# CLSFramework/gym-soccer-2d-env

Hardware: AMD Instinct MI355X
Metric: env-steps/sec at 65536 parallel reach_ball envs per MI355X (higher is better)
Workload: dtype f32

## Files before the change

gym-soccer-2d-env_amd/csrc/s2d_device.h:

```cpp
#pragma once
#include <hip/hip_runtime.h>
#include <stdint.h>

#include "../../include/s2d.h"

#define S2D_DEV __device__ __forceinline__

enum { S2D_MODE_DISCRETE = 0, S2D_MODE_CONT1 = 1, S2D_MODE_TURN4 = 2 };

struct S2DHot {
  float inv_half_l, inv_half_w, half_l, half_w;
  float player_decay, ball_decay;
  float player_accel_max2, player_speed_max2, ball_speed_max2, rsum2;
  float stamina_max, stamina_inc_max, extra_stamina, stamina_capacity;
  float recover_init, recover_dec_thr_value, recover_min, recover_dec;
  float effort_init, effort_dec_thr_value, effort_min, effort_dec, effort_inc_thr_value, effort_inc;
  float dash_power_rate, max_dash_power, min_dash_power, max_dash_angle, min_dash_angle;
  float dash_angle_step, inv_dash_angle_step, side_dash_rate, back_dash_rate;
  float min_distance_to_ball, min_dist2_thr, act_scale;
  int max_steps, n_actions, auto_reset;
  uint32_t seed_lo, seed_hi, gid_lo, gid_hi;
  float max_moment, min_moment, inertia_moment, player_rand, ball_rand;
};
struct S2DRare {
  float player_accel_max, player_speed_max, ball_speed_max, rsum, collision_vel_rate;
  float recover_init;
  float ball_position_x, ball_position_y, ball_speed, ball_direction, travel_factor;
  int change_ball_position, change_ball_velocity;
  int tab_len;
  float tab_power;
  int pad[1];
};

S2D_DEV float to_vgpr(float x) {
  float y;
  asm("v_mov_b32 %0, %1" : "=v"(y) : "s"(x));
  return y;
}
S2D_DEV S2DHot hot_in_vgprs(const S2DHot& p) {
  S2DHot v = p;
  v.inv_half_l = to_vgpr(p.inv_half_l); v.inv_half_w = to_vgpr(p.inv_half_w);
  v.half_l = to_vgpr(p.half_l); v.half_w = to_vgpr(p.half_w);
  v.player_decay = to_vgpr(p.player_decay); v.ball_decay = to_vgpr(p.ball_decay);
  v.player_accel_max2 = to_vgpr(p.player_accel_max2); v.player_speed_max2 = to_vgpr(p.player_speed_max2);
  v.ball_speed_max2 = to_vgpr(p.ball_speed_max2); v.rsum2 = to_vgpr(p.rsum2);
  v.stamina_max = to_vgpr(p.stamina_max); v.stamina_inc_max = to_vgpr(p.stamina_inc_max);
  v.extra_stamina = to_vgpr(p.extra_stamina);
  v.recover_dec_thr_value = to_vgpr(p.recover_dec_thr_value); v.recover_min = to_vgpr(p.recover_min);
  v.recover_dec = to_vgpr(p.recover_dec);
  v.effort_init = to_vgpr(p.effort_init); v.effort_dec_thr_value = to_vgpr(p.effort_dec_thr_value);
  v.effort_min = to_vgpr(p.effort_min); v.effort_dec = to_vgpr(p.effort_dec);
  v.effort_inc_thr_value = to_vgpr(p.effort_inc_thr_value); v.effort_inc = to_vgpr(p.effort_inc);
  v.dash_power_rate = to_vgpr(p.dash_power_rate); v.max_dash_power = to_vgpr(p.max_dash_power);
  v.min_dash_power = to_vgpr(p.min_dash_power); v.max_dash_angle = to_vgpr(p.max_dash_angle);
  v.min_dash_angle = to_vgpr(p.min_dash_angle);
  v.inv_dash_angle_step = to_vgpr(p.inv_dash_angle_step);
  v.side_dash_rate = to_vgpr(p.side_dash_rate); v.back_dash_rate = to_vgpr(p.back_dash_rate);
  v.min_distance_to_ball = to_vgpr(p.min_distance_to_ball); v.act_scale = to_vgpr(p.act_scale);
  v.min_dist2_thr = to_vgpr(p.min_dist2_thr);
  return v;
}

enum { S2D_ST_RESET = 0, S2D_ST_POLICY = 1, S2D_ST_SELECT = 2, S2D_ST_NOISE = 3, S2D_ST_NOISE_RESET = 5 };

struct U4 { uint32_t x, y, z, w; };

S2D_DEV U4 philox4x32_10(uint32_t c0, uint32_t c1, uint32_t c2, uint32_t c3, uint32_t k0, uint32_t k1) {
#pragma unroll
  for (int r = 0; r < 10; ++r) {
    uint64_t p0 = (uint64_t)0xD2511F53u * c0;
    uint64_t p1 = (uint64_t)0xCD9E8D57u * c2;
    uint32_t n0 = (uint32_t)(p1 >> 32) ^ c1 ^ k0, n2 = (uint32_t)(p0 >> 32) ^ c3 ^ k1;
    c0 = n0; c1 = (uint32_t)p1; c2 = n2; c3 = (uint32_t)p0;
    k0 += 0x9E3779B9u; k1 += 0xBB67AE85u;
  }
  return U4{c0, c1, c2, c3};
}
S2D_DEV U4 s2d_draw(const S2DHot& p, uint32_t gid_lo, uint32_t gid_hi, uint32_t cycle, uint32_t stream,
                    uint32_t block) {
  return philox4x32_10(gid_lo, gid_hi, cycle, (stream << 16) | block, p.seed_lo, p.seed_hi);
}
S2D_DEV U4 policy_quad(const S2DHot& p, uint32_t gid_lo, uint32_t gid_hi, uint32_t k, uint32_t stream) {
  return s2d_draw(p, gid_lo, gid_hi, k >> 2, stream, 0);
}
S2D_DEV uint32_t quad_word(const U4& q, uint32_t k) {
  uint32_t j = k & 3u;
  uint32_t lo = (j & 1u) ? q.y : q.x, hi = (j & 1u) ? q.w : q.z;
  return (j & 2u) ? hi : lo;
// ... 198 lines not shown
  }
}

S2D_DEV int command_code(float x) {
  int c = S2D_CMD_NONE;
  c = (x >= -1.5f && x <= -0.5f) ? (int)S2D_CMD_FREEZE : c;
  c = (x >= 0.5f && x < 1.5f) ? (int)S2D_CMD_DASH : c;
  c = (x >= 1.5f && x < 2.5f) ? (int)S2D_CMD_TURN : c;
  return c;
}

struct ObsOut { float o[S2D_OBS_DIM]; };

enum { S2D_FLAG_GOAL = 1, S2D_FLAG_OUT = 2, S2D_FLAG_TIMEOUT = 4 };

S2D_DEV int judge(const S2DHot& p, float px, float py, float d2, int step_number, float& dist) {
  dist = sqrt_cr(d2);
  int f = (dist < p.min_distance_to_ball) ? S2D_FLAG_GOAL : 0;
  f |= (fabsf(px) > p.half_l || fabsf(py) > p.half_w) ? S2D_FLAG_OUT : 0;
  f |= (step_number > p.max_steps) ? S2D_FLAG_TIMEOUT : 0;
  return f;
}
S2D_DEV int judge_sq(const S2DHot& p, float px, float py, float d2, int step_number) {
  int f = (d2 < p.min_dist2_thr) ? S2D_FLAG_GOAL : 0;
  f |= (fabsf(px) > p.half_l || fabsf(py) > p.half_w) ? S2D_FLAG_OUT : 0;
  f |= (step_number > p.max_steps) ? S2D_FLAG_TIMEOUT : 0;
  return f;
}
S2D_DEV float observe_player(const S2DHot& p, float px, float py, float body, float bx, float by, float* o) {
  float dx = bx - px, dy = by - py;
  float player_to_ball = atan2_deg(dy, dx);
  float rel = norm_deg(player_to_ball - body);
  o[0] = rel * 0.005555555555555556f;
  o[1] = body * 0.005555555555555556f;
  o[2] = px * p.inv_half_l;
  o[3] = py * p.inv_half_w;
  return rel;
}
S2D_DEV void observe_ball(const S2DHot& p, float bx, float by, float bvx, float bvy, float* o) {
  float ball_speed = hypot2(bvx, bvy);
  float ball_direction = atan2_deg(bvy, bvx);
  o[4] = bx * p.inv_half_l;
  o[5] = by * p.inv_half_w;
  o[6] = ball_speed * 0.3333333333333333f;
  o[7] = ball_direction * 0.002777777777777778f;
  o[8] = bvx * 0.3333333333333333f;
  o[9] = bvy * 0.3333333333333333f;
}
S2D_DEV float observe(const S2DHot& p, float px, float py, float body, float bx, float by, float bvx, float bvy,
                      ObsOut& ob) {
  observe_ball(p, bx, by, bvx, bvy, ob.o);
  return observe_player(p, px, py, body, bx, by, ob.o);
}
S2D_DEV float reward_of(float prev_dist, float prev_angle, float dist, float rel, int flags, int& result) {
  float r = prev_dist - dist;
  r += (fabsf(prev_angle) - fabsf(rel)) * 0.005555555555555556f;
  r = (flags & S2D_FLAG_GOAL) ? r + 10.0f : r;
  r = (flags & S2D_FLAG_OUT) ? r - -10.0f : r;
  r = (flags & S2D_FLAG_TIMEOUT) ? r - 5.0f : r;
  int res = (flags & S2D_FLAG_GOAL) ? S2D_RESULT_GOAL : S2D_RESULT_NONE;
  res = (flags & S2D_FLAG_OUT) ? S2D_RESULT_OUT : res;
  res = (flags & S2D_FLAG_TIMEOUT) ? S2D_RESULT_TIMEOUT : res;
  result = res;
  return r;
}

S2D_DEV void observe_and_check(const S2DHot& p, Env& e, float d2, ObsOut& ob, int& done, float& reward, int& result) {
  float rel = observe(p, e.px, e.py, e.body, e.bx, e.by, e.bvx, e.bvy, ob);
  float dist;
  int flags = judge(p, e.px, e.py, d2, e.step_number, dist);
  reward = reward_of(e.prev_dist, e.prev_angle, dist, rel, flags, result);
  e.prev_dist = dist;
  e.prev_angle = rel;
  done = flags ? 1 : 0;
}

struct CmdPrep { float power, dir, dir_rate; };
S2D_DEV CmdPrep dash_prepare(const S2DHot& p, float power, float dir) {
  power = clampf(power, p.min_dash_power, p.max_dash_power);
  dir = clampf(dir, p.min_dash_angle, p.max_dash_angle);
  float disc = p.dash_angle_step * rintf(dir * p.inv_dash_angle_step);
  dir = (p.dash_angle_step > 0.0f) ? disc : dir;
  float ad = fabsf(dir);
  float r_back = p.back_dash_rate - ((p.back_dash_rate - p.side_dash_rate) * (1.0f - (ad - 90.0f) * 0.011111111111111112f));
  float r_fwd = p.side_dash_rate + ((1.0f - p.side_dash_rate) * (1.0f - ad * 0.011111111111111112f));
  float dir_rate = clampf(ad > 90.0f ? r_back : r_fwd, 0.0f, 1.0f);
  return CmdPrep{power, dir, dir_rate};
}
S2D_DEV void dash_apply(const S2DHot& p, Env& e, const CmdPrep& c, float& ax, float& ay) {
  float power = c.power;
  bool back = power < 0.0f;
  float need = back ? power * -2.0f : power;
  float avail = e.stamina + p.extra_stamina;
  need = (need > avail) ? avail : need;
  float st = e.stamina - need;
  e.stamina = st > 0.0f ? st : 0.0f;
  power = back ? need / -2.0f : need;
  float acc = fabsf(e.effort * power * c.dir_rate * p.dash_power_rate);
  float dir = back ? c.dir + 180.0f : c.dir;
  float sn, cs;
  sincos_deg(norm_deg(e.body + dir), sn, cs);
  ax = acc * cs;
  ay = acc * sn;
}
S2D_DEV CmdPrep cmd_prepare(const S2DHot& p, int cmd, float power, float dir) {
  if (cmd == S2D_CMD_DASH) return dash_prepare(p, power, dir);
  return CmdPrep{power, dir, 0.0f};
}
S2D_DEV void cmd_turn(const S2DHot& p, Env& e, float moment, bool noise, float noise_u) {
  moment = clampf(moment, p.min_moment, p.max_moment);
  float speed = hypot2(e.vx, e.vy);
  float f = noise ? 1.0f + (noise_u * 2.0f - 1.0f) * p.player_rand : 1.0f;
  e.body = norm_deg(e.body + f * moment / (1.0f + p.inertia_moment * speed));
}
struct NoiseIn { float pm, ps, pc, bm, bs, bc, tu; };
struct NoiseWords { uint32_t wp, wb; float tu; };
S2D_DEV float noise_mag(uint32_t w) { return (float)(w >> 16) * 1.52587890625e-05f; }
// ... 333 lines not shown
```

gym-soccer-2d-env_amd/csrc/s2d_engine.hip:

```cpp
#include <hip/hip_runtime.h>

#include <cmath>
#include <cstdio>
#include <cstdlib>
#include <cstring>
#include <new>
#include <string>
#include <type_traits>

#include "s2d_device.h"

#include "s2d_actor_launch.h"
#include "s2d_kernels.h"

__global__ void s2d_tables_kernel(S2DHot p, const S2DRare* __restrict__ rp, S2DTables* __restrict__ t) {
  if (blockIdx.x == 0 && threadIdx.x == 0 && rp->tab_len > 0) tables_build(p, rp->recover_init, rp->tab_power, rp->tab_len, *t);
}
__global__ __launch_bounds__(kBlock) void s2d_init_kernel(S2DHot p, const S2DRare* __restrict__ rp,
                                                          float* __restrict__ S, int64_t stride, int64_t n) {
  int64_t i = (int64_t)blockIdx.x * kBlock + threadIdx.x;
  if (i >= n) return;
  S[F_STAMINA * stride + i] = p.stamina_max;
  S[F_RECOVERY * stride + i] = rp->recover_init;
  S[F_EFFORT * stride + i] = p.effort_init;
// ... 324 lines not shown
      const uint32_t k = k0 + (uint32_t)t;
      CmdPrep c;
      if (lut) {
        if (t == 0 || (k & 3u) == 0u) quad = policy_quad(p, gl, gh, k, S2D_ST_POLICY);
        const int a = (int)rnd_below(quad_word(quad, k), (uint32_t)p.n_actions);
        if (ro.action) static_cast<int32_t*>(ro.action)[row + i] = a;
        const float4 e4 = act_lut[wv][a];
        c = CmdPrep{e4.x, e4.y, e4.z}; dir = e4.w; cmd = S2D_CMD_DASH;
      } else {
        c = decide<MODE>(p, actions, kind, row + i, gl, gh, k, t == 0 || (k & 3u) == 0u, quad, squad, ro.action, cmd, dir);
      }
      if (fast) step_env<NK, true>(p, rp, e, gl, gh, k, cmd, c, ob, reward, done, res, term_row, &prep[wv], lane, have_prep, ep_lds, sc_lut);
      else step_env<NK, false>(p, rp, e, gl, gh, k, cmd, c, ob, reward, done, res, term_row, &prep[wv], lane, have_prep);
      if (ro.reward) ro.reward[row + i] = reward;
      if (ro.done) ro.done[row + i] = (uint8_t)done;
      if (ro.result) ro.result[row + i] = (uint8_t)res;
      cnt1 += res == S2D_RESULT_GOAL; cnt2 += res == S2D_RESULT_OUT; cnt3 += res == S2D_RESULT_TIMEOUT;
    }
    if (p.auto_reset) n_missing += __popcll(__ballot(active && done != 0));
    if (ro.obs) store_obs_tile(lds[wv], ob, lane, active, ro.obs + (row + wave_first) * S2D_OBS_DIM, valid);
  }
  if (active) {
    if (fast) {
      const int q = e.step_number;
      e.stamina = tb->stamina[q]; e.effort = tb->effort[q]; e.recovery = tb->recovery[q]; e.capacity = tb->capacity[q];
    }
    env_store(e, S, stride, i);
    if (use_k) kplane[i] = k0 + (uint32_t)n_steps;
    o.reward[i] = reward; o.done[i] = (uint8_t)done; o.result[i] = (uint8_t)res;
    o.action_dir[i] = dir; o.action_cmd[i] = (uint8_t)cmd;
  }
  store_obs_tile(lds[wv], ob, lane, active, o.obs + wave_first * S2D_OBS_DIM, valid);
  if (!active) { cnt1 = cnt2 = cnt3 = 0; }
#pragma unroll
  for (int off = 32; off > 0; off >>= 1) {
    cnt1 += __shfl_xor(cnt1, off); cnt2 += __shfl_xor(cnt2, off); cnt3 += __shfl_xor(cnt3, off);
  }
  unsigned long long* const srow = stats_row(o.stats, wave_first);
  stats_store(srow, lane, stats_load(srow, lane), wave_first == 0 ? (unsigned long long)n * (unsigned long long)n_steps : 0ull, cnt1, cnt2, cnt3);
}

#ifndef S2D_NPRIO_S
#define S2D_NPRIO_S 3
#endif
#ifndef S2D_NPRIO_A
#define S2D_NPRIO_A 2
#endif
#ifndef S2D_NPRIO_B
#define S2D_NPRIO_B 2
#endif
#ifndef S2D_NPRIO_P
#define S2D_NPRIO_P 1
#endif
#ifndef S2D_PRIO_S
#define S2D_PRIO_S 1
#endif
#ifndef S2D_PRIO_A
#define S2D_PRIO_A 2
#endif
#ifndef S2D_PRIO_B
#define S2D_PRIO_B 3
#endif

#ifdef S2D_STAMPS
#define WS_STAMP_DECL uint64_t st_busy = 0, st_t0 = __builtin_amdgcn_s_memtime(); const uint64_t st_begin = st_t0, st_rt0 = __builtin_amdgcn_s_memrealtime()
#define WS_BARRIER() do { st_busy += __builtin_amdgcn_s_memtime() - st_t0; __syncthreads(); st_t0 = __builtin_amdgcn_s_memtime(); } while (0)
#define WS_STAMP_STORE() do { if (lane == 0) { float* q_ = o.terminal_obs + (wave_first + 2 * role) * S2D_OBS_DIM; \
    q_[0] = (float)st_busy; q_[1] = (float)(__builtin_amdgcn_s_memtime() - st_begin); q_[2] = (float)(st_rt0 & 0xffffff); \
    q_[3] = (float)(__builtin_amdgcn_s_memrealtime() & 0xffffff); \
    q_[4] = __int_as_float((int)__builtin_amdgcn_s_getreg((31 << 11) | 4)); q_[5] = __int_as_float((int)__builtin_amdgcn_s_getreg((31 << 11) | 20)); } } while (0)
#else
#define WS_STAMP_DECL do {} while (0)
#define WS_BARRIER() __syncthreads()
#define WS_STAMP_STORE() do {} while (0)
#endif

template <int MODE, int NK, int REC = 0>
__global__ __launch_bounds__(kWsBlock, 4) void s2d_reach_rollout_ws_kernel(S2DHot p_sgpr, const S2DRare* __restrict__ rp,
                                                                        float* __restrict__ S, int64_t stride,
                                                                        int64_t n, int n_steps,
                                                                        const void* __restrict__ actions, int kind,
                                                                        RolloutOut ro, StepOut o) {
  constexpr bool NOISE = NK != S2D_NK_OFF;
  constexpr int kActWords = NOISE ? (int)WA_WORDS : (int)WA_NPM;
  __shared__ float act[3][kActWords][kWave];
  __shared__ float snap[2][WS_WORDS][kWave];
  __shared__ float slots[kSlots][SL_WORDS][kWave];
  __shared__ __attribute__((aligned(16))) float tile[2][kObsTile];
  __shared__ float4 act_lut[kWave];
  __shared__ float ep_lds[S2D_TAB_MAX];
  __shared__ float2 sc_lut[361];
  const int lane = threadIdx.x & (kWave - 1);
  const int role = __builtin_amdgcn_readfirstlane(threadIdx.x / kWave);
  const bool nt = REC == 2 || (REC == 0 && ro.nt != 0);
  const int64_t wave_first = (int64_t)blockIdx.x * kWave;
  const int64_t i = wave_first + lane;
  const bool active = i < n;
  int64_t rows = n - wave_first; rows = rows > kWave ? kWave : rows;
  const int valid = (int)rows * S2D_OBS_DIM;
  const int n_iter = n_steps + 3;

  if (role != 1 && p_sgpr.auto_reset) {
    const uint64_t gid = (((uint64_t)p_sgpr.gid_hi << 32) | p_sgpr.gid_lo) + (uint64_t)i;
    uint32_t ep0 = 0u;
    if (active) ep0 = reinterpret_cast<const uint32_t*>(S + F_EPISODE * stride)[i];
    const int k = role == 0 ? 0 : role - 1;
    slot_fill_coop<NK>(p_sgpr, rp, slots[k], lane, (uint32_t)gid, (uint32_t)(gid >> 32), ep0 + 1u + (uint32_t)k, active,
                          reinterpret_cast<uint32_t*>(&tile[0][0]) + role * kWave);
  }

  if (role == 0) {
    if constexpr (NOISE) __builtin_amdgcn_s_setprio(S2D_NPRIO_P);
    const S2DHot& p = p_sgpr;
    const bool use_k = uses_policy_step<MODE, NOISE>(kind);
    uint32_t* const kplane = reinterpret_cast<uint32_t*>(S + F_POLICY * stride);
    uint32_t gl = 0, gh = 0, k0 = 0;
    if (active) {
      if (use_k) k0 = kplane[i];
      uint64_t gid = (((uint64_t)p.gid_hi << 32) | p.gid_lo) + (uint64_t)i;
      gl = (uint32_t)gid; gh = (uint32_t)(gid >> 32);
    }
    U4 quad{0, 0, 0, 0}, squad{0, 0, 0, 0}, nblk{0, 0, 0, 0};
    float dir = 0.0f; int cmd = 0;
    int64_t row = 0;
    const bool lut = MODE == S2D_MODE_DISCRETE && kind == S2D_ACT_RANDOM && p.n_actions <= kWave;
    if (lut && lane < p.n_actions) {
      int c0; float pw, d0;
      action_map<MODE>(p, Action4{(float)lane, 0.0f, 0.0f, 0.0f}, 0.0f, c0, pw, d0);
      const CmdPrep c = cmd_prepare(p, c0, pw, d0);
      act_lut[lane] = make_float4(c.power, c.dir, c.dir_rate, d0);
    }
    __syncthreads();
    WS_STAMP_DECL;
    int wslot = 0;
    auto policy_step = [&](int t) {
      if (active) {
        const uint32_t k = k0 + (uint32_t)t;
        CmdPrep c;
        if (lut) {
          if (t == 0 || (k & 3u) == 0u) quad = policy_quad(p, gl, gh, k, S2D_ST_POLICY);
          const int a = (int)rnd_below(quad_word(quad, k), (uint32_t)p.n_actions);
          if (REC != 0 || ro.action) rec_store(static_cast<int32_t*>(ro.action) + row + i, (int32_t)a, nt);
          const float4 e4 = act_lut[a];
          c = CmdPrep{e4.x, e4.y, e4.z}; dir = e4.w; cmd = S2D_CMD_DASH;
        } else {
          c = decide<MODE>(p, actions, kind, row + i, gl, gh, k, t == 0 || (k & 3u) == 0u, quad, squad, ro.action, cmd, dir);
        }
        const int b = wslot;
        if (MODE == S2D_MODE_TURN4) act[b][WA_CMD][lane] = __int_as_float(cmd);
        act[b][WA_POWER][lane] = c.power;
        act[b][WA_DIR][lane] = c.dir; act[b][WA_RATE][lane] = c.dir_rate;
        if constexpr (NK == S2D_NK_SQUARE) {
          const NoiseIn nz = noise_prepare_square(p, gl, gh, k, S2D_ST_NOISE, cmd == S2D_CMD_TURN);
          act[b][WA_NPM][lane] = nz.pm; act[b][WA_NPS][lane] = nz.ps; act[b][WA_NPC][lane] = nz.pc;
          act[b][WA_NBM][lane] = nz.bm; act[b][WA_NBS][lane] = nz.bs; act[b][WA_NBC][lane] = nz.bc;
          if (MODE == S2D_MODE_TURN4) act[b][WA_NTU][lane] = nz.tu;
        } else if constexpr (NOISE) {
          const NoiseWords nw = noise_words(p, gl, gh, k, S2D_ST_NOISE, cmd == S2D_CMD_TURN, nblk, t == 0 || (k & 1u) == 0u);
          const float2 ps = sc_lut[noise_dir_index(nw.wp)], bs = sc_lut[noise_dir_index(nw.wb)];
          act[b][WA_NPM][lane] = noise_mag(nw.wp); act[b][WA_NPS][lane] = ps.x; act[b][WA_NPC][lane] = ps.y;
          act[b][WA_NBM][lane] = noise_mag(nw.wb); act[b][WA_NBS][lane] = bs.x; act[b][WA_NBC][lane] = bs.y;
          if (MODE == S2D_MODE_TURN4) act[b][WA_NTU][lane] = nw.tu;
        }
        row += n;
      }
      wslot = wslot == 2 ? 0 : wslot + 1;
    };
    for (int s = 0; s < n_iter; ++s) {
      if (s == 0 && n_steps > 0) policy_step(0);
      if (s + 1 < n_steps) policy_step(s + 1);
      WS_BARRIER();
    }
    WS_STAMP_STORE();
    if (active) {
      if (use_k) kplane[i] = k0 + (uint32_t)n_steps;
      o.action_dir[i] = dir; o.action_cmd[i] = (uint8_t)cmd;
    }
  } else if (role == 1) {
    if constexpr (NOISE) __builtin_amdgcn_s_setprio(S2D_NPRIO_S);
    else __builtin_amdgcn_s_setprio(S2D_PRIO_S);
    const S2DHot p = hot_in_vgprs(p_sgpr);
    Env e;
    uint32_t gl = 0, gh = 0;
    int nth = 0, j = 0;
    if (active) {
      env_load(e, S, stride, i);
      uint64_t gid = (((uint64_t)p.gid_hi << 32) | p.gid_lo) + (uint64_t)i;
      gl = (uint32_t)gid; gh = (uint32_t)(gid >> 32);
      asm volatile("" ::"v"(e.px), "v"(e.py), "v"(e.vx), "v"(e.vy), "v"(e.body), "v"(e.stamina), "v"(e.effort),
                   "v"(e.recovery), "v"(e.capacity), "v"(e.bx), "v"(e.by), "v"(e.bvx), "v"(e.bvy),
                   "v"(e.step_number), "v"(e.cycle), "v"(e.episode));
    }
    const S2DTables* const tb = tables_of(rp);
    const int tab_len = MODE != S2D_MODE_TURN4 ? rp->tab_len : 0;
    bool fast = false;
    if (tab_len > 0) {
      bool ok = true;
      if (active) {
        const int sn = e.step_number;
        ok = sn >= 0 && sn < tab_len;
        const int q = ok ? sn : 0;
        ok = ok && e.stamina == tb->stamina[q] && e.effort == tb->effort[q] && e.recovery == tb->recovery[q] &&
             e.capacity == tb->capacity[q] && e.body == rintf(e.body) && fabsf(e.body) <= 180.0f;
      }
      fast = __ballot(active && !ok) == 0ull;
      if (fast)
        for (int k = lane; k < tab_len; k += kWave) ep_lds[k] = tb->ep[k];
    }
    if (fast || NK == S2D_NK_LATTICE) {
      for (int k = lane; k <= 360; k += kWave) {
        float sn, cs;
        sincos_deg((float)(k - 180), sn, cs);
        sc_lut[k] = make_float2(sn, cs);
      }
    }
    const ResetStamina rst = reset_stamina(p, rp);
    __syncthreads();
    WS_STAMP_DECL;
    auto loop = [&](auto fast_tag) {
      constexpr bool FAST = decltype(fast_tag)::value;
      struct ActRegs { float cmd, power, dir, rate, npm, nps, npc, nbm, nbs, nbc, ntu; };
      ActRegs cur{}, nxt{};
      float ep_cur = 0.0f; float2 sc_cur = make_float2(0.0f, 0.0f);
      int rslot = 1;
      auto fetch = [&](int slot) {
        ActRegs r{};
        if (MODE == S2D_MODE_TURN4) r.cmd = act[slot][WA_CMD][lane];
        if (!FAST) r.power = act[slot][WA_POWER][lane];
        r.dir = act[slot][WA_DIR][lane]; r.rate = act[slot][WA_RATE][lane];
        if constexpr (NOISE) {
          r.npm = act[slot][WA_NPM][lane]; r.nps = act[slot][WA_NPS][lane]; r.npc = act[slot][WA_NPC][lane];
          r.nbm = act[slot][WA_NBM][lane]; r.nbs = act[slot][WA_NBS][lane]; r.nbc = act[slot][WA_NBC][lane];
          if (MODE == S2D_MODE_TURN4) r.ntu = act[slot][WA_NTU][lane];
// ... 24 lines not shown
          if constexpr (FAST) {
            e.step_number += 1;
            d2 = sim_cycle_dash_fast<NOISE>(p, rp, e, ep_cur, cur.rate, sc_cur.x, sc_cur.y, nz);
          } else {
            const CmdPrep c{cur.power, cur.dir, cur.rate};
            e.step_number += 1;
            d2 = sim_cycle<NOISE, true>(p, rp, e, cmd, c, nz);
          }
          int flags = judge_sq(p, e.px, e.py, d2, e.step_number);
          const bool took = flags && p.auto_reset;
          snap[b][WS_PX][lane] = e.px; snap[b][WS_PY][lane] = e.py; snap[b][WS_BODY][lane] = e.body;
          snap[b][WS_BX][lane] = e.bx; snap[b][WS_BY][lane] = e.by;
          snap[b][WS_BVX][lane] = e.bvx; snap[b][WS_BVY][lane] = e.bvy;
          snap[b][WS_FLAGS][lane] = __int_as_float(flags | (j << 8));
          if (took) {
            if (nth >= kSlots)
              slot_fill<NK>(p, rp, slots[j], lane, gl, gh, (uint32_t)e.episode + 1u);
            episode_begin(e, slot_take<kWave>(slots[j], lane, rst));
            nth += 1; j = (j + 1 == kSlots) ? 0 : j + 1;
          }
          if (more) { cur = nxt; lookups(); }
        }
        if (STEADY || (s >= 1 && s < n_steps)) rslot = rslot == 2 ? 0 : rslot + 1;
        WS_BARRIER();
      };
      int s = 0;
      for (; s < 2 && s < n_iter; ++s) simulate_iteration(s, std::false_type{});
      for (; s < n_steps; ++s) simulate_iteration(s, std::true_type{});
      for (; s < n_iter; ++s) simulate_iteration(s, std::false_type{});
    };
    if (fast) {
      loop(std::true_type{});
      if (active) {
        const int q = e.step_number;
        e.stamina = tb->stamina[q]; e.effort = tb->effort[q]; e.recovery = tb->recovery[q]; e.capacity = tb->capacity[q];
      }
    } else {
      loop(std::false_type{});
    }
    WS_STAMP_STORE();
    if (active) {
      S[F_PX * stride + i] = e.px; S[F_PY * stride + i] = e.py;
      S[F_VX * stride + i] = e.vx; S[F_VY * stride + i] = e.vy;
      S[F_BODY * stride + i] = e.body;
      S[F_STAMINA * stride + i] = e.stamina; S[F_EFFORT * stride + i] = e.effort;
      S[F_RECOVERY * stride + i] = e.recovery; S[F_CAPACITY * stride + i] = e.capacity;
      S[F_BX * stride + i] = e.bx; S[F_BY * stride + i] = e.by;
      S[F_BVX * stride + i] = e.bvx; S[F_BVY * stride + i] = e.bvy;
      S[F_STEP * stride + i] = __int_as_float(e.step_number);
      S[F_CYCLE * stride + i] = __int_as_float(e.cycle);
      S[F_EPISODE * stride + i] = __int_as_float(e.episode);
    }
  } else if (role == 2) {
    __builtin_amdgcn_s_setprio(NOISE ? S2D_NPRIO_A : S2D_PRIO_A);
    const S2DHot p = hot_in_vgprs(p_sgpr);
    const bool auto_reset = p_sgpr.auto_reset != 0;
    float prev_dist = 0.0f, prev_angle = 0.0f;
    if (active) {
      prev_dist = S[F_PREV_DIST * stride + i]; prev_angle = S[F_PREV_ANGLE * stride + i];
      asm volatile("" ::"v"(prev_dist), "v"(prev_angle));
    }
    float oa[S2D_OBS_DIM];
    float reward = 0.0f; int res = 0, done = 0;
    unsigned int cnt1 = 0, cnt2 = 0, cnt3 = 0;
    unsigned long long* const srow = stats_row(o.stats, wave_first);
    const unsigned long long sold = stats_load(srow, lane);
    float* const term_row = o.terminal_obs + i * S2D_OBS_DIM;
    int64_t row = 0;
    __syncthreads();
    WS_STAMP_DECL;
    auto agent_iteration = [&](int s, auto steady_tag) {
      constexpr bool STEADY = decltype(steady_tag)::value;
      if (STEADY || (s >= 2 && s < n_steps + 2)) {
        const int b = s & 1;
        res = 0;
        if (active) {
          float px = snap[b][WS_PX][lane], py = snap[b][WS_PY][lane], body = snap[b][WS_BODY][lane];
          float bx = snap[b][WS_BX][lane], by = snap[b][WS_BY][lane];
          const int fw = __float_as_int(snap[b][WS_FLAGS][lane]);
          const int flags = fw & 0xff;
          float dist = hypot2(bx - px, by - py);
          float rel = observe_player(p, px, py, body, bx, by, oa);
          reward = reward_of(prev_dist, prev_angle, dist, rel, flags, res);
          prev_dist = dist; prev_angle = rel;
          done = flags ? 1 : 0;
          if (flags && auto_reset) {
            const float (*sl)[kWave] = slots[fw >> 8];
#pragma unroll
            for (int k = 0; k < 4; ++k) term_row[k] = oa[k];
#pragma unroll
            for (int k = 0; k < 4; ++k) oa[k] = sl[SL_FIRST + k][lane];
            prev_dist = sl[SL_DIST][lane]; prev_angle = sl[SL_REL][lane];
          }
          if (REC != 0 || ro.reward) rec_store(ro.reward + row + i, reward, nt);
          if (REC != 0 || ro.done) rec_store(ro.done + row + i, (uint8_t)done, nt);
          if (REC != 0 || ro.result) rec_store(ro.result + row + i, (uint8_t)res, nt);
          cnt1 += res == S2D_RESULT_GOAL; cnt2 += res == S2D_RESULT_OUT; cnt3 += res == S2D_RESULT_TIMEOUT;
          if (REC != 0 || ro.obs) {
            float* t = &tile[b][lane * S2D_OBS_DIM];
            t[0] = oa[0]; t[1] = oa[1]; t[2] = oa[2]; t[3] = oa[3];
          }
        }
        row += n;
      }
      WS_BARRIER();
    };
    {
      int s = 0;
      for (; s < 3 && s < n_iter; ++s) agent_iteration(s, std::false_type{});
      for (; s < n_steps + 2; ++s) agent_iteration(s, std::true_type{});
      for (; s < n_iter; ++s) agent_iteration(s, std::false_type{});
    }
    WS_STAMP_STORE();
    if (active) {
      S[F_PREV_DIST * stride + i] = prev_dist; S[F_PREV_ANGLE * stride + i] = prev_angle;
      o.reward[i] = reward; o.done[i] = (uint8_t)done; o.result[i] = (uint8_t)res;
#pragma unroll
      for (int k = 0; k < 4; ++k) o.obs[i * S2D_OBS_DIM + k] = oa[k];
    }
    if (!active) { cnt1 = cnt2 = cnt3 = 0; }
#pragma unroll
    for (int off = 32; off > 0; off >>= 1) {
      cnt1 += __shfl_xor(cnt1, off); cnt2 += __shfl_xor(cnt2, off); cnt3 += __shfl_xor(cnt3, off);
    }
    stats_store(srow, lane, sold, wave_first == 0 ? (unsigned long long)n * (unsigned long long)n_steps : 0ull, cnt1, cnt2, cnt3);
  } else {
    if constexpr (NOISE) __builtin_amdgcn_s_setprio(S2D_NPRIO_B);
    else __builtin_amdgcn_s_setprio(S2D_PRIO_B);
    const S2DHot p = hot_in_vgprs(p_sgpr);
    const bool auto_reset = p_sgpr.auto_reset != 0;
    float ob6[S2D_OBS_DIM];
    float* const term_row = o.terminal_obs + i * S2D_OBS_DIM;
    const bool obs_all_vec = valid == kObsTile && ((n * S2D_OBS_DIM * 4) & 15) == 0 &&
                             (reinterpret_cast<uintptr_t>(ro.obs + wave_first * S2D_OBS_DIM) & 15u) == 0;
    __syncthreads();
    WS_STAMP_DECL;
    auto ball_iteration = [&](int s, auto steady_tag) {
      constexpr bool STEADY = decltype(steady_tag)::value;
      if ((STEADY || s >= 3) && (REC != 0 || ro.obs))
        tile_flush(tile[(s - 1) & 1], lane, ro.obs + ((int64_t)(s - 3) * n + wave_first) * S2D_OBS_DIM, valid, nt, obs_all_vec);
      if ((STEADY || (s >= 2 && s < n_steps + 2)) && active) {
        const int b = s & 1;
        float bx = snap[b][WS_BX][lane], by = snap[b][WS_BY][lane];
        float bvx = snap[b][WS_BVX][lane], bvy = snap[b][WS_BVY][lane];
        const int fw = __float_as_int(snap[b][WS_FLAGS][lane]);
        observe_ball(p, bx, by, bvx, bvy, ob6);
        if ((fw & 0xff) && auto_reset) {
          const float (*sl)[kWave] = slots[fw >> 8];
#pragma unroll
          for (int k = 4; k < S2D_OBS_DIM; ++k) term_row[k] = ob6[k];
#pragma unroll
          for (int k = 4; k < S2D_OBS_DIM; ++k) ob6[k] = sl[SL_FIRST + k][lane];
        }
        if (REC != 0 || ro.obs) {
          float* t = &tile[b][lane * S2D_OBS_DIM];
#pragma unroll
          for (int k = 4; k < S2D_OBS_DIM; ++k) t[k] = ob6[k];
        }
      }
      WS_BARRIER();
    };
    {
      int s = 0;
      for (; s < 3 && s < n_iter; ++s) ball_iteration(s, std::false_type{});
      for (; s < n_steps + 2; ++s) ball_iteration(s, std::true_type{});
      for (; s < n_iter; ++s) ball_iteration(s, std::false_type{});
    }
    WS_STAMP_STORE();
    if (active) {
#pragma unroll
      for (int k = 4; k < S2D_OBS_DIM; ++k) o.obs[i * S2D_OBS_DIM + k] = ob6[k];
    }
  }
}

__global__ __launch_bounds__(kBlock) void s2d_world_model_kernel(const float* __restrict__ S, int64_t stride,
                                                                 int64_t n, S2DWorldModel w) {
  int64_t i = (int64_t)blockIdx.x * kBlock + threadIdx.x;
  if (i >= n) return;
  float px = S[F_PX * stride + i], py = S[F_PY * stride + i], vx = S[F_VX * stride + i], vy = S[F_VY * stride + i];
  float bx = S[F_BX * stride + i], by = S[F_BY * stride + i], bvx = S[F_BVX * stride + i], bvy = S[F_BVY * stride + i];
// ... 523 lines not shown
  hipLaunchKernelGGL(table[h->mode][h->nk], dim3(main_blocks + refill_blocks), dim3(kBlock), 0,
                     static_cast<hipStream_t>(stream), h->hot, h->rare_dev, reinterpret_cast<float*>(h->buf.player_x), h->stride, h->n,
                     k, actions_dev, action_kind, ro, h->out, refill_blocks);
  HIP_TRY(hipGetLastError());
  h->last_kernel = "s2d_reach_step_k_kernel";
  return S2D_OK;
}

S2D_API int s2d_rollout(S2DHandle h, int n_steps, const void* actions_dev, int action_kind, const S2DRollout* out,
                        void* stream) {
  if (!h) return fail(S2D_EINVAL, "NULL handle");
  if (n_steps < 0) return fail(S2D_EINVAL, "n_steps must be >= 0");
  if (action_kind == S2D_ACT_COMMAND) return fail(S2D_EINVAL, "S2D_ACT_COMMAND is a per-step action kind (s2d_step)");
  int rc = check_action_kind(h, actions_dev, action_kind);
  if (rc != S2D_OK) return rc;
  if (n_steps == 0) return S2D_OK;
  RolloutOut ro{nullptr, nullptr, nullptr, nullptr, nullptr, 0};
  if (out) {
    ro = RolloutOut{out->obs, out->action, out->reward, out->done, out->result, 0};
    const int64_t per_step = (out->obs ? 4 * S2D_OBS_DIM : 0) + (out->action ? (h->mode == S2D_MODE_TURN4 ? 16 : 4) : 0) + (out->reward ? 4 : 0) + (out->done ? 1 : 0) +
                             (out->result ? 1 : 0);
    ro.nt = h->rollout_nt >= 0 ? h->rollout_nt : ((int64_t)n_steps * h->n * per_step > kInfinityCacheBytes);
    if (h->cfg.task.use_continuous_action && h->cfg.task.use_turning && (reinterpret_cast<uintptr_t>(out->action) & 15u))
      return fail(S2D_EINVAL, "rollout action buffer float[T][N][4] must be 16-byte aligned");
    if (reinterpret_cast<uintptr_t>(out->obs) & 3u) return fail(S2D_EINVAL, "rollout obs buffer must be 4-byte aligned");
  }
  DeviceGuard guard(h->device);
  using RollK = void (*)(S2DHot, const S2DRare*, float*, int64_t, int64_t, int, const void*, int, RolloutOut, StepOut);
  static const RollK table[3][3] = {
      {s2d_reach_rollout_kernel<S2D_MODE_DISCRETE, S2D_NK_OFF>, s2d_reach_rollout_kernel<S2D_MODE_DISCRETE, S2D_NK_LATTICE>,
       s2d_reach_rollout_kernel<S2D_MODE_DISCRETE, S2D_NK_SQUARE>},
      {s2d_reach_rollout_kernel<S2D_MODE_CONT1, S2D_NK_OFF>, s2d_reach_rollout_kernel<S2D_MODE_CONT1, S2D_NK_LATTICE>,
       s2d_reach_rollout_kernel<S2D_MODE_CONT1, S2D_NK_SQUARE>},
      {s2d_reach_rollout_kernel<S2D_MODE_TURN4, S2D_NK_OFF>, s2d_reach_rollout_kernel<S2D_MODE_TURN4, S2D_NK_LATTICE>,
       s2d_reach_rollout_kernel<S2D_MODE_TURN4, S2D_NK_SQUARE>}};
  static const RollK table_ws[3][3] = {
      {s2d_reach_rollout_ws_kernel<S2D_MODE_DISCRETE, S2D_NK_OFF>, s2d_reach_rollout_ws_kernel<S2D_MODE_DISCRETE, S2D_NK_LATTICE>,
       s2d_reach_rollout_ws_kernel<S2D_MODE_DISCRETE, S2D_NK_SQUARE>},
      {s2d_reach_rollout_ws_kernel<S2D_MODE_CONT1, S2D_NK_OFF>, s2d_reach_rollout_ws_kernel<S2D_MODE_CONT1, S2D_NK_LATTICE>,
       s2d_reach_rollout_ws_kernel<S2D_MODE_CONT1, S2D_NK_SQUARE>},
      {s2d_reach_rollout_ws_kernel<S2D_MODE_TURN4, S2D_NK_OFF>, s2d_reach_rollout_ws_kernel<S2D_MODE_TURN4, S2D_NK_LATTICE>,
       s2d_reach_rollout_ws_kernel<S2D_MODE_TURN4, S2D_NK_SQUARE>}};
  const bool ws = h->rollout_ws < 0 ? (h->n <= kWsMaxEnvs) : (h->rollout_ws != 0);
  static const char* const mode_names[3] = {"discrete", "continuous", "turning"};
  if (ws) {
    if (h->rollout_e == 2 && h->nk != S2D_NK_SQUARE && s2d_internal_rollout2(h->mode, h->noise ? 1 : 0, &h->hot, h->rare_dev, reinterpret_cast<float*>(h->buf.player_x),
                                                   h->stride, h->n, n_steps, actions_dev, action_kind, &ro, &h->out, stream, h->kernel_name)) {
      HIP_TRY(hipGetLastError());
      h->last_kernel = h->kernel_name;
      return S2D_OK;
    }
    RollK kern_ws = table_ws[h->mode][h->nk];
    int rec = 0;
    if (h->mode == S2D_MODE_DISCRETE && !h->noise && ro.obs && ro.action && ro.reward && ro.done && ro.result) {
      kern_ws = ro.nt ? s2d_reach_rollout_ws_kernel<S2D_MODE_DISCRETE, S2D_NK_OFF, 2> : s2d_reach_rollout_ws_kernel<S2D_MODE_DISCRETE, S2D_NK_OFF, 1>;
      rec = ro.nt ? 2 : 1;
    }
    hipLaunchKernelGGL(kern_ws, dim3((unsigned)((h->n + kWave - 1) / kWave)),
                       dim3(kWsBlock), 0, static_cast<hipStream_t>(stream), h->hot, h->rare_dev,
                       reinterpret_cast<float*>(h->buf.player_x), h->stride, h->n, n_steps, actions_dev, action_kind,
                       ro, h->out);
    HIP_TRY(hipGetLastError());
    std::snprintf(h->kernel_name, sizeof h->kernel_name, "s2d_reach_rollout_ws_kernel<%s,noise=%d,rec=%d,nt=%d>", mode_names[h->mode],
                  h->nk, rec, ro.nt ? 1 : 0);
    h->last_kernel = h->kernel_name;
    return S2D_OK;
  }
  hipLaunchKernelGGL(table[h->mode][h->nk], dim3(grid_for(h->n)), dim3(kBlock), 0,
                     static_cast<hipStream_t>(stream), h->hot, h->rare_dev,
                     reinterpret_cast<float*>(h->buf.player_x), h->stride, h->n, n_steps, actions_dev, action_kind,
                     ro, h->out);
  HIP_TRY(hipGetLastError());
  std::snprintf(h->kernel_name, sizeof h->kernel_name, "s2d_reach_rollout_kernel<%s,noise=%d>", mode_names[h->mode], h->nk);
  h->last_kernel = h->kernel_name;
  return S2D_OK;
}


static int actor_fail(const char* who, const char* what) { return fail(S2D_EINVAL, std::string(who) + what); }

static int actor_begin(const char* who, S2DEngine* h, const void* net, unsigned modes, const char* wrong_mode, int n_steps,
                       const S2DRollout* out, const float* terminal_obs, const float* logp, RolloutOut& ro) {
  const auto misaligned = [](const void* q, unsigned m) { return (reinterpret_cast<uintptr_t>(q) & m) != 0; };
  if (!h) return fail(S2D_EINVAL, "NULL handle");
  if (!net) return actor_fail(who, ": net is NULL");
  if (!(modes >> h->mode & 1u)) return fail(S2D_EINVAL, wrong_mode);
  if (n_steps < 1) return actor_fail(who, ": n_steps must be >= 1");
  if (misaligned(terminal_obs, 3u)) return actor_fail(who, ": terminal_obs must be 4-byte aligned");
  if (misaligned(logp, 3u)) return actor_fail(who, ": logp must be 4-byte aligned");
  ro = RolloutOut{nullptr, nullptr, nullptr, nullptr, nullptr, 0};
  if (out) {
    ro = RolloutOut{out->obs, out->action, out->reward, out->done, out->result, 0};
    if (misaligned(out->obs, 3u)) return fail(S2D_EINVAL, "rollout obs buffer must be 4-byte aligned");
    if (misaligned(out->action, h->mode == S2D_MODE_TURN4 ? 15u : 3u))
      return fail(S2D_EINVAL, modes >> S2D_MODE_TURN4 & 1u ? "rollout action buffer must be 4-byte (16-byte on a turning engine) aligned"
                                                         : "rollout action buffer must be 4-byte aligned");
  }
  return S2D_OK;
}

static int actor_pointers(const char* who, const float* params, const float* epsilon, const float* noise, int noise_kind,
                          int max_noise_kind) {
  const auto bad = [](const void* q, unsigned m) { return !q || (reinterpret_cast<uintptr_t>(q) & m) != 0; };
  if (noise_kind < 0 || noise_kind > max_noise_kind)
    return actor_fail(who, max_noise_kind ? ": noise_kind must be 0 (none) or 1 (Gaussian)"
                                          : ": noise_kind must be 0 (the Q actor has no action noise)");
  if (bad(params, 15u)) return actor_fail(who, ": params must be a non-NULL, 16-byte aligned device pointer");
  if (bad(epsilon, 3u)) return actor_fail(who, ": epsilon must be a non-NULL, 4-byte aligned device pointer");
  if (noise_kind == 1 && bad(noise, 3u)) return actor_fail(who, ": Gaussian noise needs a non-NULL, 4-byte aligned noise buffer [2][n_out]");
  return S2D_OK;
}

static int actor_n_out(const char* who, const S2DEngine* h, int n_out) {
  const bool turn = h->mode == S2D_MODE_TURN4;
  if (n_out == (turn ? 4 : 1)) return S2D_OK;
  return actor_fail(who, turn ? ": n_out must be 4 on a turning engine" : ": n_out must be 1 on a continuous (non-turning) engine");
}
// ... 213 lines not shown
```

Measured before the change: 105.9 billion.

## Add LUT-based random-policy producer wave and skip terminal reward work when no lane finishes

Adds a PLUT specialization of the warp-specialized rollout kernel for discrete, noise-free, fully recorded random-action runs. The policy wave fills a per-wave lookup table of prepared dash commands once, then each step only draws the Philox random action and copies that table entry into shared memory, avoiding per-step action mapping and command preparation. Wave priorities are retuned for this variant. The reward wave now splits the terminal bonus and episode-result counting into a branch that runs only when some lane in the wave has terminal flags, which removes that work on most steps at the cost of an extra ballot.

```diff
diff --git a/gym-soccer-2d-env_amd/csrc/s2d_device.h b/gym-soccer-2d-env_amd/csrc/s2d_device.h
--- a/gym-soccer-2d-env_amd/csrc/s2d_device.h
+++ b/gym-soccer-2d-env_amd/csrc/s2d_device.h
@@ -34,6 +34,11 @@
 
 S2D_DEV float to_vgpr(float x) {
   float y;
+  asm("v_mov_b32 %0, %1" : "=v"(y) : "s"(x));
+  return y;
+}
+S2D_DEV uint32_t to_vgpr(uint32_t x) {
+  uint32_t y;
   asm("v_mov_b32 %0, %1" : "=v"(y) : "s"(x));
   return y;
 }
@@ -338,9 +343,12 @@
   observe_ball(p, bx, by, bvx, bvy, ob.o);
   return observe_player(p, px, py, body, bx, by, ob.o);
 }
-S2D_DEV float reward_of(float prev_dist, float prev_angle, float dist, float rel, int flags, int& result) {
+S2D_DEV float reward_base(float prev_dist, float prev_angle, float dist, float rel) {
   float r = prev_dist - dist;
   r += (fabsf(prev_angle) - fabsf(rel)) * 0.005555555555555556f;
+  return r;
+}
+S2D_DEV float reward_terminal(float r, int flags, int& result) {
   r = (flags & S2D_FLAG_GOAL) ? r + 10.0f : r;
   r = (flags & S2D_FLAG_OUT) ? r - -10.0f : r;
   r = (flags & S2D_FLAG_TIMEOUT) ? r - 5.0f : r;
@@ -349,6 +357,9 @@
   res = (flags & S2D_FLAG_TIMEOUT) ? S2D_RESULT_TIMEOUT : res;
   result = res;
   return r;
+}
+S2D_DEV float reward_of(float prev_dist, float prev_angle, float dist, float rel, int flags, int& result) {
+  return reward_terminal(reward_base(prev_dist, prev_angle, dist, rel), flags, result);
 }
 
 S2D_DEV void observe_and_check(const S2DHot& p, Env& e, float d2, ObsOut& ob, int& done, float& reward, int& result) {
diff --git a/gym-soccer-2d-env_amd/csrc/s2d_engine.hip b/gym-soccer-2d-env_amd/csrc/s2d_engine.hip
--- a/gym-soccer-2d-env_amd/csrc/s2d_engine.hip
+++ b/gym-soccer-2d-env_amd/csrc/s2d_engine.hip
@@ -400,6 +400,15 @@
 #ifndef S2D_NPRIO_P
 #define S2D_NPRIO_P 1
 #endif
+#ifndef S2D_LPRIO_S
+#define S2D_LPRIO_S 3
+#endif
+#ifndef S2D_LPRIO_A
+#define S2D_LPRIO_A 1
+#endif
+#ifndef S2D_LPRIO_B
+#define S2D_LPRIO_B 2
+#endif
 #ifndef S2D_PRIO_S
 #define S2D_PRIO_S 1
 #endif
@@ -423,7 +432,7 @@
 #define WS_STAMP_STORE() do {} while (0)
 #endif
 
-template <int MODE, int NK, int REC = 0>
+template <int MODE, int NK, int REC = 0, bool PLUT = false>
 __global__ __launch_bounds__(kWsBlock, 4) void s2d_reach_rollout_ws_kernel(S2DHot p_sgpr, const S2DRare* __restrict__ rp,
                                                                         float* __restrict__ S, int64_t stride,
                                                                         int64_t n, int n_steps,
@@ -457,7 +466,54 @@
                           reinterpret_cast<uint32_t*>(&tile[0][0]) + role * kWave);
   }
 
-  if (role == 0) {
+  if constexpr (PLUT) {
+    static_assert(!PLUT || (MODE == S2D_MODE_DISCRETE && !NOISE && REC != 0), "PLUT: discrete actions, noise off, the whole record");
+  }
+  if (PLUT && role == 0) {
+    uint32_t* const kplane = reinterpret_cast<uint32_t*>(S + F_POLICY * stride);
+    uint32_t gl = 0, gh = 0, k0 = 0;
+    if (active) {
+      k0 = kplane[i];
+      const uint64_t gid = (((uint64_t)p_sgpr.gid_hi << 32) | p_sgpr.gid_lo) + (uint64_t)i;
+      gl = (uint32_t)gid; gh = (uint32_t)(gid >> 32);
+    }
+    if (lane < p_sgpr.n_actions) {
+      int c0; float pw, d0;
+      action_map<MODE>(p_sgpr, Action4{(float)lane, 0.0f, 0.0f, 0.0f}, 0.0f, c0, pw, d0);
+      const CmdPrep c = cmd_prepare(p_sgpr, c0, pw, d0);
+      act_lut[lane] = make_float4(c.power, c.dir, c.dir_rate, d0);
+    }
+    const uint32_t seed_lo = to_vgpr(p_sgpr.seed_lo), seed_hi = to_vgpr(p_sgpr.seed_hi), span = to_vgpr((uint32_t)p_sgpr.n_actions);
+    __syncthreads();
+    WS_STAMP_DECL;
+    U4 quad{0, 0, 0, 0};
+    float dir = 0.0f;
+    int32_t* arow = static_cast<int32_t*>(ro.action) + i;
+    int wslot = 0;
+    auto policy_step = [&](int t, auto first_tag) {
+      if (active) {
+        const uint32_t k = k0 + (uint32_t)t;
+        if (decltype(first_tag)::value || (k & 3u) == 0u)
+          quad = philox4x32_10(gl, gh, k >> 2, (uint32_t)S2D_ST_POLICY << 16, seed_lo, seed_hi);
+        const int a = rnd_below(quad_word(quad, k), span);
+        rec_store(arow, (int32_t)a, nt);
+        const float4 e4 = act_lut[a];
+        act[wslot][WA_POWER][lane] = e4.x; act[wslot][WA_DIR][lane] = e4.y; act[wslot][WA_RATE][lane] = e4.z;
+        dir = e4.w;
+        arow += n;
+      }
+      wslot = wslot == 2 ? 0 : wslot + 1;
+    };
+    policy_step(0, std::true_type{});
+    int s = 0;
+    for (; s + 1 < n_steps; ++s) { policy_step(s + 1, std::false_type{}); WS_BARRIER(); }
+    for (; s < n_iter; ++s) WS_BARRIER();
+    WS_STAMP_STORE();
+    if (active) {
+      kplane[i] = k0 + (uint32_t)n_steps;
+      o.action_dir[i] = dir; o.action_cmd[i] = (uint8_t)S2D_CMD_DASH;
+    }
+  } else if (role == 0) {
     if constexpr (NOISE) __builtin_amdgcn_s_setprio(S2D_NPRIO_P);
     const S2DHot& p = p_sgpr;
     const bool use_k = uses_policy_step<MODE, NOISE>(kind);
@@ -526,7 +582,7 @@
     }
   } else if (role == 1) {
     if constexpr (NOISE) __builtin_amdgcn_s_setprio(S2D_NPRIO_S);
-    else __builtin_amdgcn_s_setprio(S2D_PRIO_S);
+    else __builtin_amdgcn_s_setprio(PLUT ? S2D_LPRIO_S : S2D_PRIO_S);
     const S2DHot p = hot_in_vgprs(p_sgpr);
     Env e;
     uint32_t gl = 0, gh = 0;
@@ -657,7 +713,7 @@
       S[F_EPISODE * stride + i] = __int_as_float(e.episode);
     }
   } else if (role == 2) {
-    __builtin_amdgcn_s_setprio(NOISE ? S2D_NPRIO_A : S2D_PRIO_A);
+    __builtin_amdgcn_s_setprio(NOISE ? S2D_NPRIO_A : PLUT ? S2D_LPRIO_A : S2D_PRIO_A);
     const S2DHot p = hot_in_vgprs(p_sgpr);
     const bool auto_reset = p_sgpr.auto_reset != 0;
     float prev_dist = 0.0f, prev_angle = 0.0f;
@@ -684,23 +740,27 @@
           float bx = snap[b][WS_BX][lane], by = snap[b][WS_BY][lane];
           const int fw = __float_as_int(snap[b][WS_FLAGS][lane]);
           const int flags = fw & 0xff;
+          float rel = observe_player(p, px, py, body, bx, by, oa);
           float dist = hypot2(bx - px, by - py);
-          float rel = observe_player(p, px, py, body, bx, by, oa);
-          reward = reward_of(prev_dist, prev_angle, dist, rel, flags, res);
+          reward = reward_base(prev_dist, prev_angle, dist, rel);
           prev_dist = dist; prev_angle = rel;
-          done = flags ? 1 : 0;
-          if (flags && auto_reset) {
-            const float (*sl)[kWave] = slots[fw >> 8];
-#pragma unroll
-            for (int k = 0; k < 4; ++k) term_row[k] = oa[k];
-#pragma unroll
-            for (int k = 0; k < 4; ++k) oa[k] = sl[SL_FIRST + k][lane];
-            prev_dist = sl[SL_DIST][lane]; prev_angle = sl[SL_REL][lane];
+          done = 0;
+          if (__ballot(flags != 0) != 0ull) {
+            reward = reward_terminal(reward, flags, res);
+            done = flags ? 1 : 0;
+            if (flags && auto_reset) {
+              const float (*sl)[kWave] = slots[fw >> 8];
+#pragma unroll
+              for (int k = 0; k < 4; ++k) term_row[k] = oa[k];
+#pragma unroll
+              for (int k = 0; k < 4; ++k) oa[k] = sl[SL_FIRST + k][lane];
+              prev_dist = sl[SL_DIST][lane]; prev_angle = sl[SL_REL][lane];
+            }
+            cnt1 += res == S2D_RESULT_GOAL; cnt2 += res == S2D_RESULT_OUT; cnt3 += res == S2D_RESULT_TIMEOUT;
           }
           if (REC != 0 || ro.reward) rec_store(ro.reward + row + i, reward, nt);
           if (REC != 0 || ro.done) rec_store(ro.done + row + i, (uint8_t)done, nt);
           if (REC != 0 || ro.result) rec_store(ro.result + row + i, (uint8_t)res, nt);
-          cnt1 += res == S2D_RESULT_GOAL; cnt2 += res == S2D_RESULT_OUT; cnt3 += res == S2D_RESULT_TIMEOUT;
           if (REC != 0 || ro.obs) {
             float* t = &tile[b][lane * S2D_OBS_DIM];
             t[0] = oa[0]; t[1] = oa[1]; t[2] = oa[2]; t[3] = oa[3];
@@ -731,7 +791,7 @@
     stats_store(srow, lane, sold, wave_first == 0 ? (unsigned long long)n * (unsigned long long)n_steps : 0ull, cnt1, cnt2, cnt3);
   } else {
     if constexpr (NOISE) __builtin_amdgcn_s_setprio(S2D_NPRIO_B);
-    else __builtin_amdgcn_s_setprio(S2D_PRIO_B);
+    else __builtin_amdgcn_s_setprio(PLUT ? S2D_LPRIO_B : S2D_PRIO_B);
     const S2DHot p = hot_in_vgprs(p_sgpr);
     const bool auto_reset = p_sgpr.auto_reset != 0;
     float ob6[S2D_OBS_DIM];
@@ -1361,8 +1421,11 @@
     }
     RollK kern_ws = table_ws[h->mode][h->nk];
     int rec = 0;
+    bool plut = false;
     if (h->mode == S2D_MODE_DISCRETE && !h->noise && ro.obs && ro.action && ro.reward && ro.done && ro.result) {
-      kern_ws = ro.nt ? s2d_reach_rollout_ws_kernel<S2D_MODE_DISCRETE, S2D_NK_OFF, 2> : s2d_reach_rollout_ws_kernel<S2D_MODE_DISCRETE, S2D_NK_OFF, 1>;
+      plut = action_kind == S2D_ACT_RANDOM && h->hot.n_actions <= kWave;
+      if (plut) kern_ws = ro.nt ? s2d_reach_rollout_ws_kernel<S2D_MODE_DISCRETE, S2D_NK_OFF, 2, true> : s2d_reach_rollout_ws_kernel<S2D_MODE_DISCRETE, S2D_NK_OFF, 1, true>;
+      else kern_ws = ro.nt ? s2d_reach_rollout_ws_kernel<S2D_MODE_DISCRETE, S2D_NK_OFF, 2> : s2d_reach_rollout_ws_kernel<S2D_MODE_DISCRETE, S2D_NK_OFF, 1>;
       rec = ro.nt ? 2 : 1;
     }
     hipLaunchKernelGGL(kern_ws, dim3((unsigned)((h->n + kWave - 1) / kWave)),
@@ -1370,8 +1433,8 @@
                        reinterpret_cast<float*>(h->buf.player_x), h->stride, h->n, n_steps, actions_dev, action_kind,
                        ro, h->out);
     HIP_TRY(hipGetLastError());
-    std::snprintf(h->kernel_name, sizeof h->kernel_name, "s2d_reach_rollout_ws_kernel<%s,noise=%d,rec=%d,nt=%d>", mode_names[h->mode],
-                  h->nk, rec, ro.nt ? 1 : 0);
+    std::snprintf(h->kernel_name, sizeof h->kernel_name, "s2d_reach_rollout_ws_kernel<%s,noise=%d,rec=%d,nt=%d,plut=%d>", mode_names[h->mode],
+                  h->nk, rec, ro.nt ? 1 : 0, plut ? 1 : 0);
     h->last_kernel = h->kernel_name;
     return S2D_OK;
   }
```

Measured after the change: 107.9 billion (median of 6 runs). +1.9%, better.
